# TUI-NICR/nicr-multitask-scene-analysis

Hardware: AMD Instinct MI355X
Metric: Mpix/s panoptic merge+metrics, 640x480xB (higher is better)
Workload: dtype f32; 1 GPU; configs[1]: center-NMS + offset grouping + panoptic merge + mIoU/PQ accumulators (configs[3]); batch_per_gpu=32, global_batch=32, classes=40, height=480, width=640, centers_per_image=24, batches_in_flight=2, parallelism=dp1 (images sharded, accumulators all-reduced once per run, timed)

## Files before the change

include/nmsa.h:

```cpp
#ifndef NMSA_H
#define NMSA_H

#include <stddef.h>
#include <stdint.h>

#ifdef __cplusplus
extern "C" {
#endif

typedef void* nmsa_stream_t;

enum {
    NMSA_OK = 0,
    NMSA_ERR_ARG = -1,
    NMSA_ERR_LAUNCH = -2,
    NMSA_ERR_WORKSPACE = -3,
    NMSA_ERR_UNSUPPORTED = -4
};

enum { NMSA_F32 = 0, NMSA_BF16 = 1, NMSA_F16 = 2 };
enum { NMSA_U8 = 0, NMSA_I16 = 1, NMSA_I32 = 2, NMSA_I64 = 3 };
#define NMSA_ELEM_F32 8

#define NMSA_MAX_INSTANCE_IDS 256

int nmsa_version(void);
const char* nmsa_strerror(int code);
int nmsa_last_hip_error(void);
int nmsa_device_geometry(int* cus_host, int* xcds_host, size_t* lds_per_cu_host);

size_t nmsa_center_nms_workspace_bytes(int B, int H, int W);
int nmsa_center_nms_topk(const float* center, const uint8_t* fg,
                         int B, int H, int W,
                         float threshold, int ksize, int topk, int apply_fg,
                         int max_centers,
                         int32_t* centers_yx, int32_t* n_centers, float* scores,
                         uint8_t* center_mask,
                         void* workspace, size_t workspace_bytes,
                         nmsa_stream_t stream);

int nmsa_group_offsets(const float* offset, const uint8_t* fg,
                       const int32_t* centers_yx, const int32_t* n_centers,
                       int B, int H, int W, int max_centers,
                       float scale_y, float scale_x,
                       int use_dist_thr, float dist_thr,
                       uint8_t* inst, int32_t* area,
                       nmsa_stream_t stream);

int nmsa_semantic_argmax(const void* logits, int logits_dtype,
                         int B, int C, int H, int W,
                         uint8_t* idx_u8, int64_t* idx_i64, float* score,
                         nmsa_stream_t stream);

int nmsa_semantic_softmax(const void* logits, int logits_dtype,
                          int B, int C, int H, int W, float* probs,
                          nmsa_stream_t stream);

int nmsa_panoptic_fused(const void* logits, int logits_dtype, const float* offset,
                        const int32_t* centers_yx, const int32_t* n_centers,
                        const uint8_t* is_thing,
                        int B, int C, int H, int W, int max_centers,
                        float scale_y, float scale_x,
                        int use_dist_thr, float dist_thr,
                        uint8_t* sem_u8, uint8_t* inst, uint8_t* fg_out, float* score,
                        uint32_t* votes, int votes_are_zero, int vote_rows_hint,
                        nmsa_stream_t stream);

int nmsa_panoptic_assign(uint32_t* votes, int B, int n_vote_classes, int clear_votes,
                         int64_t max_instances_per_category, int64_t void_label,
                         int64_t* pan_of_inst, int32_t* area,
                         int64_t* ids_pan, int64_t* ids_ins, int32_t* n_ids,
                         nmsa_stream_t stream);

int nmsa_panoptic_paint(const uint8_t* sem_u8, const uint8_t* inst,
                        const int64_t* pan_of_inst, const uint8_t* is_thing,
                        int B, int C, int H, int W,
                        int64_t max_instances_per_category, int64_t void_label,
                        int64_t* pan, int64_t* pan_sem,
                        nmsa_stream_t stream);

int nmsa_panoptic_merge(const void* sem, int sem_dtype, const void* ins, int ins_dtype,
                        const uint8_t* thing_seg, const uint8_t* is_thing_class,
                        int B, int n_classes, int H, int W,
                        int64_t max_instances_per_category, int64_t void_label,
                        uint32_t* votes, int64_t* pan_of_inst,
                        int64_t* pan, int64_t* ids_pan, int64_t* ids_ins, int32_t* n_ids,
                        nmsa_stream_t stream);

size_t nmsa_panoptic_merge_wide_workspace_bytes(int B, int n_classes, int max_segments);
int nmsa_panoptic_merge_wide(const void* sem, int sem_dtype, const void* ins, int ins_dtype,
                             const uint8_t* thing_seg, const uint8_t* is_thing_class,
                             int B, int n_classes, int H, int W,
// ... 387 lines not shown
```

nicr_mt_scene_analysis_amd/_lib.py:

```python
import ctypes as C
import os
import re
import subprocess
from typing import Optional

import torch

_HERE = os.path.dirname(os.path.abspath(__file__))
CSRC_DIR = os.path.join(_HERE, 'csrc')
LIB_PATH = os.environ.get('NMSA_LIB_PATH') or os.path.join(CSRC_DIR, 'libnmsa_hip.so')
HEADER_PATH = os.path.join(os.path.dirname(_HERE), 'include', 'nmsa.h')

NMSA_F32, NMSA_BF16, NMSA_F16 = 0, 1, 2
NMSA_U8, NMSA_I16, NMSA_I32, NMSA_I64 = 0, 1, 2, 3
NMSA_ST_VALUE_RANGE = 8
NMSA_SCENE_MAX_CLASSES = 4096
(NMSA_TG_ROUTE_SCAN, NMSA_TG_ROUTE_FAST_LOADERS, NMSA_TG_ROUTE_PAINT_TILED, NMSA_TG_ROUTE_PAINT_VECTOR,
 NMSA_TG_ROUTE_LUT_LDS, NMSA_TG_ROUTE_SCAN_16) = 1, 2, 4, 8, 16, 32
NMSA_UP_ROUTE_VECTOR, NMSA_UP_ROUTE_PIXEL = 1, 2
NMSA_LNT_ROUTE_VECTOR, NMSA_LNT_ROUTE_ELEMENT = 1, 2
NMSA_LNT_MAX_CHANNELS = 2048


class NmsaError(RuntimeError):
    pass


def build(force: bool = False) -> str:
    args = ['make', '-C', CSRC_DIR, '-j4']
    if force:
        args.append('-B')
    subprocess.check_call(args, stdout=subprocess.DEVNULL)
    return LIB_PATH


def declared_symbols():
    with open(HEADER_PATH) as f:
        text = f.read()
    text = re.sub(r'/\*.*?\*/', '', text, flags=re.S)
    return sorted(set(re.findall(r'\b(nmsa_[a-z0-9_]+)\s*\(', text)))


_vp, _i, _f, _i64, _sz = C.c_void_p, C.c_int, C.c_float, C.c_int64, C.c_size_t

_SIGNATURES = {
    'nmsa_version': (C.c_int, []),
    'nmsa_strerror': (C.c_char_p, [_i]),
    'nmsa_last_hip_error': (C.c_int, []),
    'nmsa_device_geometry': (_i, [_vp, _vp, _vp]),
    'nmsa_center_nms_workspace_bytes': (_sz, [_i, _i, _i]),
    'nmsa_center_nms_topk': (_i, [_vp, _vp, _i, _i, _i, _f, _i, _i, _i, _i,
                                  _vp, _vp, _vp, _vp, _vp, _sz, _vp]),
    'nmsa_group_offsets': (_i, [_vp, _vp, _vp, _vp, _i, _i, _i, _i, _f, _f, _i, _f,
                                _vp, _vp, _vp]),
    'nmsa_semantic_argmax': (_i, [_vp, _i, _i, _i, _i, _i, _vp, _vp, _vp, _vp]),
    'nmsa_semantic_softmax': (_i, [_vp, _i, _i, _i, _i, _i, _vp, _vp]),
    'nmsa_panoptic_fused': (_i, [_vp, _i, _vp, _vp, _vp, _vp, _i, _i, _i, _i, _i,
                                 _f, _f, _i, _f, _vp, _vp, _vp, _vp, _vp, _i, _i, _vp]),
    'nmsa_panoptic_assign': (_i, [_vp, _i, _i, _i, _i64, _i64, _vp, _vp, _vp, _vp, _vp, _vp]),
    'nmsa_panoptic_paint': (_i, [_vp, _vp, _vp, _vp, _i, _i, _i, _i, _i64, _i64,
                                 _vp, _vp, _vp]),
    'nmsa_panoptic_merge': (_i, [_vp, _i, _vp, _i, _vp, _vp, _i, _i, _i, _i, _i64, _i64,
                                 _vp, _vp, _vp, _vp, _vp, _vp, _vp]),
    'nmsa_panoptic_merge_wide_workspace_bytes': (_sz, [_i, _i, _i]),
    'nmsa_panoptic_merge_wide': (_i, [_vp, _i, _vp, _i, _vp, _vp, _i, _i, _i, _i, _i64, _i64, _i,
                                      _vp, _vp, _vp, _vp, _vp, _vp, _sz, _vp]),
    'nmsa_resize_nearest': (_i, [_vp, _i, _i, _i, _i, _i, _i, _i, _i, _i, _i, _vp, _vp]),
    'nmsa_resize_bilinear': (_i, [_vp, _i, _i, _i, _i, _i, _i, _i, _i, _i, _i, _vp, _vp]),
    'nmsa_semantic_argmax_resized': (_i, [_vp, _i, _i, _i, _i, _i, _i, _i, _i, _i, _i, _i,
                                          _vp, _vp, _vp, _vp]),
    'nmsa_panoptic_scores_workspace_bytes': (_sz, [_i]),
    'nmsa_panoptic_scores': (_i, [_vp, _i, _vp, _vp, _vp, _vp, _vp, _vp, _i, _i, _i, _i, _i64,
                                  _vp, _vp, _vp, _vp, _vp, _sz, _vp]),
    'nmsa_targets_workspace_bytes': (_sz, [_i, _i, _i]),
    'nmsa_targets_route': (_i, [_vp, _i, _vp, _i, _i, _i, _i, _i, _i, _vp, _vp, _vp, _vp, _vp]),
    'nmsa_instance_clear_stuff': (_i, [_vp, _i, _vp, _i, _vp, _i, _i64, _vp]),
    'nmsa_instance_targets': (_i, [_vp, _i, _vp, _i, _vp, _vp, _i, _i, _i, _i, _i, _vp, _i, _i,
                                   _vp, _vp, _vp, _vp, _vp, _vp, _vp, _vp, _vp, _vp, _sz, _i, _vp]),
    'nmsa_panoptic_targets': (_i, [_vp, _i, _vp, _i, _vp, _i, _i, _i, _i, _i64, _i64, _i, _i,
                                   _vp, _vp, _vp, _vp, _vp, _vp, _sz, _i, _vp]),
    'nmsa_orientation_targets': (_i, [_vp, _i, _vp, _i, _vp, _vp, _vp, _vp, _i, _i, _i, _i, _i, _i,
                                      _vp, _vp, _vp, _vp, _vp, _sz, _i, _vp]),
    'nmsa_dve_targets': (_i, [_vp, _vp, _vp, _vp, _vp, _f, _i, _i, _i, _i, _i, _vp, _vp, _vp]),
    'nmsa_dve_project': (_i, [_vp, _i, _i, _i, _i, _vp, _i, _vp, _vp, _i, _vp, _i, _vp]),
    'nmsa_dve_project_route': (_i, [_vp, _i, _i, _i, _i, _vp, _i, _vp, _vp, _i, _vp, _i]),
    'nmsa_normal_valid_mask': (_i, [_vp, _i, _i, _i, _vp, _vp]),
    'nmsa_rmse_update': (_i, [_vp, _i, _vp, _vp, _i, _i, _i, _i, _i, _i, _i, _i, _i, _i, _i,
                              _vp, _vp, _vp]),
    'nmsa_maae_update_keyed': (_i, [_vp, _vp, _vp, _vp, _i, _vp, _vp, _vp, _vp, _vp, _i, _vp,
                                    _i, _vp, _vp, _vp, _vp]),
    'nmsa_maae_update_matched': (_i, [_vp, _vp, _i, _vp, _vp, _vp, _i, _i, _vp, _vp, _vp, _vp, _i, _vp,
                                      _vp, _vp, _vp, _i, _i, _vp, _vp, _vp, _vp, _i, _vp,
                                      _i, _vp, _vp, _vp, _vp]),
    'nmsa_multiscale_nearest': (_i, [_vp, _vp, _i, _i, _vp]),
    'nmsa_batch_augment': (_i, [_vp, _vp, _i, _i, _i, _vp]),
    'nmsa_scene_step': (_i, [_vp, _i, _vp, _i, _i, _i, _vp, _f, _vp, _vp, _vp, _vp, _vp, _vp, _vp]),
    'nmsa_upsample2x_dw3x3_route': (_i, [_vp, _vp, _i, _i, _i, _i, _i]),
    'nmsa_upsample2x_dw3x3_fwd': (_i, [_vp, _i, _vp, _vp, _i, _i, _i, _i, _i, _vp, _vp]),
    'nmsa_upsample2x_dw3x3_bwd_workspace_bytes': (_sz, [_i, _i, _i, _i]),
    'nmsa_upsample2x_dw3x3_bwd': (_i, [_vp, _vp, _i, _vp, _i, _i, _i, _i, _i, _vp, _vp, _vp, _vp, _sz, _vp]),
    'nmsa_ln_nhwc_nchw_route': (_i, [_vp, _vp, _i, _i, _i, _i, _i]),
    'nmsa_ln_nhwc_nchw_fwd': (_i, [_vp, _i, _vp, _vp, _f, _vp, _i, _i, _i, _vp, _i, _vp, _vp, _vp]),
    'nmsa_ln_nhwc_nchw_bwd_workspace_bytes': (_sz, [_i, _i, _i]),
    'nmsa_ln_nhwc_nchw_bwd': (_i, [_vp, _i, _vp, _i, _vp, _vp, _vp, _i, _i, _i, _vp, _vp, _vp, _vp, _sz, _vp]),
    'nmsa_instance_orientation_wide': (_i, [_vp, _vp, _i, _vp, _i, _i, _i, _i, _vp, _vp, _vp, _vp,
# ... 4 lines not shown
    'nmsa_pq_confmat_workspace_bytes': (_sz, [_i, _i, _i, _i]),
    'nmsa_pq_update_with_confmat': (_i, [_vp, _vp, _vp, _i, _i, _i, _i, _i64, _i64, _i64, _i64,
                                         _vp, _vp, _vp, _vp, _vp, _i, _vp, _vp, _vp, _sz, _i,
                                         _i, _i64, _vp, _vp, _vp, _sz, _vp]),
    'nmsa_pq_update_with_confmat_parts': (_i, [_vp, _vp, _vp, _vp, _i, _i64, _vp, _vp, _i, _i, _i,
                                               _i, _i64, _i64, _i64, _i64, _vp, _vp, _vp, _vp,
                                               _vp, _vp, _sz, _i, _i, _i64, _vp, _vp, _vp, _sz, _vp]),
    'nmsa_pack_tables': (_i, [_vp, _vp, _vp, _vp, _vp, _vp, _vp, _i, _i, _i, _vp, _vp]),
    'nmsa_loss_workspace_bytes': (_sz, [_i, _i, _i]),
    'nmsa_loss_ce_fwd': (_i, [_vp, _i, _vp, _vp, _i, _i, _i, _i, _f, _vp, _vp, _vp, _vp, _vp, _vp, _sz,
                              _vp]),
    'nmsa_loss_ce_bwd': (_i, [_vp, _i, _vp, _vp, _i, _i, _i, _i, _f, _vp, _vp, _vp, _vp]),
    'nmsa_loss_ce_fwd_i16': (_i, [_vp, _i, _vp, _vp, _i, _i, _i, _i, _f, _vp, _vp, _vp, _vp, _vp, _vp, _sz,
                                  _vp]),
    'nmsa_loss_ce_bwd_i16': (_i, [_vp, _i, _vp, _vp, _i, _i, _i, _i, _f, _vp, _vp, _vp, _vp]),
    'nmsa_loss_masked_fwd': (_i, [_vp, _i, _vp, _vp, _i, _i, _i, _i, _i, _vp, _vp, _vp, _sz, _vp]),
    'nmsa_loss_masked_bwd': (_i, [_vp, _i, _vp, _vp, _i, _i, _i, _i, _i, _vp, _vp, _vp]),
    'nmsa_loss_vonmises_fwd': (_i, [_vp, _i, _vp, _vp, _i, _i, _i, _f, _vp, _vp, _vp, _sz, _vp]),
    'nmsa_loss_vonmises_bwd': (_i, [_vp, _i, _vp, _vp, _i, _i, _i, _f, _vp, _vp, _vp]),
    'nmsa_loss_ce_fwd_grad_supported': (_i, [_i, _i]),
    'nmsa_loss_ce_fwd_grad': (_i, [_vp, _i, _vp, _vp, _i, _i, _i, _i, _f, _vp, _vp, _vp, _vp, _vp, _vp,
                                   _vp, _sz, _vp]),
    'nmsa_loss_ce_bwd_unless': (_i, [_vp, _i, _vp, _vp, _i, _i, _i, _i, _f, _vp, _vp, _vp, _vp, _vp]),
    'nmsa_count_workspace_bytes': (_sz, []),
    'nmsa_count_u8': (_i, [_vp, _i64, _i, _i, _vp, _vp, _f, _vp, _sz, _vp]),
    'nmsa_loss_cos_emb_fwd_grad_supported': (_i, [_i, _i, _i, _i, _i]),
    'nmsa_loss_cos_emb_fwd_grad_workspace_bytes': (_sz, [_i, _i, _i, _i, _i]),
    'nmsa_loss_cos_emb_fwd_grad': (_i, [_vp, _i, _vp, _vp, _i, _i, _i, _i, _i, _vp, _vp, _vp, _vp, _vp, _vp, _sz, _vp]),
    'nmsa_loss_cos_emb_bwd_unless': (_i, [_vp, _i, _vp, _vp, _i, _i, _i, _i, _i, _vp, _vp, _vp, _vp, _vp, _sz, _vp]),
    'nmsa_multitask_loss_workspace_bytes': (_sz, [_vp, _i]),
    'nmsa_multitask_loss_fwd_grad': (_i, [_vp, _i, _i, _vp, _vp, _vp, _vp, _vp, _vp, _vp, _vp, _sz, _vp]),
    'nmsa_multitask_loss_bwd_unless': (_i, [_vp, _i, _i, _vp, _vp, _vp, _vp, _vp, _vp, _vp, _vp, _vp, _sz, _vp]),
    'nmsa_loss_masked_fwd_grad': (_i, [_vp, _i, _vp, _vp, _i, _i, _i, _i, _i, _vp, _vp, _vp, _vp, _vp,
                                       _sz, _vp]),
    'nmsa_loss_masked_bwd_unless': (_i, [_vp, _i, _vp, _vp, _i, _i, _i, _i, _i, _vp, _vp, _vp, _vp,
                                         _vp]),
    'nmsa_loss_vonmises_fwd_grad': (_i, [_vp, _i, _vp, _vp, _i, _i, _i, _f, _vp, _vp, _vp, _vp, _vp,
                                         _sz, _vp]),
    'nmsa_loss_vonmises_bwd_unless': (_i, [_vp, _i, _vp, _vp, _i, _i, _i, _f, _vp, _vp, _vp, _vp, _vp]),
    'nmsa_loss_cos_emb_fwd': (_i, [_vp, _i, _vp, _vp, _i, _i, _i, _i, _i, _vp, _vp, _vp, _vp, _vp, _sz, _vp]),
    'nmsa_loss_cos_emb_bwd': (_i, [_vp, _i, _vp, _vp, _i, _i, _i, _i, _i, _vp, _vp, _vp, _vp]),
    'nmsa_loss_cos_emb_can_keep_dots': (_i, [_i, _i, _i, _i]),
    'nmsa_loss_elementwise_none_fwd': (_i, [_vp, _i, _vp, _i64, _i, _i, _vp, _vp]),
    'nmsa_loss_elementwise_none_bwd': (_i, [_vp, _i, _vp, _i64, _i, _i, _vp, _vp, _vp]),
    'nmsa_loss_cos_rows_fwd': (_i, [_vp, _i, _vp, _vp, _i64, _i, _f, _vp, _vp]),
    'nmsa_loss_cos_rows_bwd': (_i, [_vp, _i, _vp, _vp, _i64, _i, _f, _vp, _i, _vp, _vp]),
    'nmsa_loss_vonmises_rows_fwd': (_i, [_vp, _i, _vp, _i64, _f, _vp, _vp]),
    'nmsa_loss_vonmises_rows_bwd': (_i, [_vp, _i, _vp, _i64, _f, _vp, _vp, _vp]),
    'nmsa_pq_workspace_bytes': (_sz, [_i, _i, _i, _i]),
    'nmsa_pq_update': (_i, [_vp, _vp, _i, _i, _i, _i, _i64, _i64, _i64, _i64,
                            _vp, _vp, _vp, _vp, _vp, _i, _vp, _vp, _vp, _sz, _i, _vp]),
}

_lib = None


def lib():
    global _lib
    if _lib is None:
        if not os.path.exists(LIB_PATH):
            raise NmsaError(
                f'{LIB_PATH} is missing: the HIP extension was not built. Run '
                '`python -c "import __graft_entry__ as g; g.build()"` '
                '(or `make -C nicr_mt_scene_analysis_amd/csrc`). There is no '
                'CPU/PyTorch fallback for this path.')
        handle = C.CDLL(LIB_PATH)
        for name, (res, args) in _SIGNATURES.items():
            fn = getattr(handle, name)
            fn.restype = res
            fn.argtypes = args
        _lib = handle
    return _lib


def check(rc: int, what: str) -> None:
    if rc != 0:
        l_ = lib()
        msg = l_.nmsa_strerror(rc).decode()
        hip = l_.nmsa_last_hip_error()
        raise NmsaError(f'{what}: {msg} (code {rc}, hipError {hip})')


def device_geometry():
    cus, xcds, lds = C.c_int(0), C.c_int(0), C.c_size_t(0)
    check(lib().nmsa_device_geometry(C.byref(cus), C.byref(xcds), C.byref(lds)), 'nmsa_device_geometry')
    return cus.value, xcds.value, lds.value


def ptr(t: Optional[torch.Tensor]):
    if t is None:
        return None
    if not t.is_cuda and not t.is_pinned():
        raise ValueError(f'the C-ABI takes device (or pinned host) memory; got a pageable '
                         f'{t.device} tensor of shape {tuple(t.shape)}')
    return C.c_void_p(t.data_ptr())


def stream_ptr(device) -> C.c_void_p:
    return C.c_void_p(torch.cuda.current_stream(device).cuda_stream)


def float_dtype_code(t: torch.Tensor) -> int:
    if t.dtype == torch.float32:
        return NMSA_F32
    if t.dtype == torch.bfloat16:
        return NMSA_BF16
    if t.dtype == torch.float16:
        return NMSA_F16
    raise TypeError(f'unsupported floating dtype {t.dtype}')


def int_dtype_code(t: torch.Tensor) -> int:
    if t.dtype in (torch.uint8, torch.bool):
        return NMSA_U8
    if t.dtype == torch.int16:
        return NMSA_I16
    if t.dtype == torch.int32:
        return NMSA_I32
    if t.dtype == torch.int64:
        return NMSA_I64
# ... 10 lines not shown
```

nicr_mt_scene_analysis_amd/csrc/center_nms.hip:

```cpp
#include <stdlib.h>
#include "nmsa_common.hpp"

namespace nmsa {

constexpr int NMS_TW = 64;
constexpr int NMS_TH = 16;
constexpr int NMS_PAD_MAX = 4;

__device__ __forceinline__ float threshold_m1(float x, float thr)
{
    return (x <= thr) ? -1.0f : x;
}

template <bool USE_LDS>
__global__ __launch_bounds__(256) void k_nms_candidates(
    const float* __restrict__ center, uint32_t* __restrict__ cand_bits,
    int H, int W, int words_per_image, float thr, int pad)
{
    __shared__ float tile[USE_LDS ? (NMS_TH + 2 * NMS_PAD_MAX) * (NMS_TW + 2 * NMS_PAD_MAX) : 1];
    const int b = blockIdx.z;
    const int x0 = blockIdx.x * NMS_TW, y0 = blockIdx.y * NMS_TH;
    const float* img = center + (size_t)b * H * W;
    const int tw = NMS_TW + 2 * pad, th = NMS_TH + 2 * pad;

// ... 80 lines not shown
    uint32_t* bits = cand_bits + (size_t)b * words_per_image;
    constexpr int K = 2 * PAD + 1;
    for (int xb = 0; xb < W; xb += blockDim.x) {
        const int x = xb + threadIdx.x;
        const bool in_x = x < W;
        const int xc = in_x ? x : 0;
        float win[K][K];
#pragma unroll
        for (int i = 0; i < K - 1; ++i)
#pragma unroll
            for (int j = 0; j < K; ++j)
                win[i + 1][j] = strip[i * tw + xc + j];
        for (int r = 0; r < rows; ++r) {
            const int y = y0 + r;
#pragma unroll
            for (int i = 0; i < K - 1; ++i)
#pragma unroll
                for (int j = 0; j < K; ++j) win[i][j] = win[i + 1][j];
#pragma unroll
            for (int j = 0; j < K; ++j) win[K - 1][j] = strip[(r + K - 1) * tw + xc + j];
            bool cand = false;
            if (in_x) {
                const float h = win[PAD][PAD];
                bool survive;
                if (y < PAD || y >= H - PAD || x < PAD || x >= W - PAD) {
                    survive = (y * W + x == 0) && (h == 0.0f);
                } else {
                    survive = true;
#pragma unroll
                    for (int i = 0; i < K; ++i)
#pragma unroll
                        for (int j = 0; j < K; ++j) {
                            if (i == PAD && j == PAD) continue;
                            const bool before = (i < PAD) || (i == PAD && j < PAD);
                            survive = survive && (before ? (win[i][j] < h) : (win[i][j] <= h));
                        }
                    survive = survive && (h == h);
                }
                cand = survive && h >= 0.0f;
            }
            const unsigned long long m = __ballot(cand);
            if (lane_id() == 0) {
                const int x_wave = xb + (int)(threadIdx.x & ~63u);
                if (x_wave < W) {
                    const int word = (y * W + x_wave) >> 5;
                    bits[word] = (uint32_t)m;
                    if (x_wave + 32 < W) bits[word + 1] = (uint32_t)(m >> 32);
                }
            }
        }
    }
}


template <int NR_ROWS, bool HALF>
__global__ __launch_bounds__(256) void k_nms_rows3(
    const float* __restrict__ center, uint32_t* __restrict__ cand_bits,
    int H, int W, int words_per_image, float thr, int blocks_per_image, int n_blocks, int n_xcd)
{
    constexpr int LPB = HALF ? 32 : 64;
    constexpr int BW = LPB * 4;
    const int per_xcd = n_blocks > 0 ? (n_blocks + n_xcd - 1) / n_xcd : 0;
    const int logical = n_blocks > 0 ? (int)(blockIdx.x % n_xcd) * per_xcd + (int)(blockIdx.x / n_xcd) : (int)blockIdx.x;
    if (n_blocks > 0 && logical >= n_blocks) return;
    const int b = n_blocks > 0 ? logical / blocks_per_image : (int)blockIdx.y;
    const int bx = n_blocks > 0 ? logical - b * blocks_per_image : (int)blockIdx.x;
    const int lane = lane_id();
    const int l = lane & (LPB - 1);
    const int sub = HALF ? (lane >> 5) : 0;
    const int bands = (W + BW - 1) / BW;
    const int wave = bx * 4 + (int)(threadIdx.x >> 6);
    const int seg = wave / bands, band = wave - seg * bands;
    const int y0 = (seg * (HALF ? 2 : 1) + sub) * NR_ROWS;
    if ((seg * (HALF ? 2 : 1)) * NR_ROWS >= H) return;
    const int xb = band * BW;
    const int x0 = xb + 4 * l;
    const bool in_x = x0 < W && y0 < H;
    const float* img = center + (size_t)b * H * W;
    const int xe = (l == 0) ? xb - 1 : xb + BW;
    const bool edge_lane = (l == 0 || l == LPB - 1) && xe >= 0 && xe < W;

    float4 row[NR_ROWS + 2];
    float edge[NR_ROWS + 2];
#pragma unroll
    for (int r = 0; r < NR_ROWS + 2; ++r) {
        const int gy = min(max(y0 - 1 + r, 0), H - 1);
        row[r] = in_x ? *(const float4*)(img + (size_t)gy * W + x0) : make_float4(-1.f, -1.f, -1.f, -1.f);
        edge[r] = edge_lane ? img[(size_t)gy * W + xe] : -1.f;
    }
    auto extend = [&](int r, float e[6]) {
        const float4 v = row[r];
        e[1] = threshold_m1(v.x, thr); e[2] = threshold_m1(v.y, thr);
        e[3] = threshold_m1(v.z, thr); e[4] = threshold_m1(v.w, thr);
        const float ev = threshold_m1(edge[r], thr);
        const float lf = __shfl_up(e[4], 1), rr = __shfl_down(e[1], 1);
        e[0] = (l == 0) ? ev : lf;
        e[5] = (l == LPB - 1) ? ev : rr;
    };
    uint32_t* bits = cand_bits + (size_t)b * words_per_image;
    auto hmax3 = [](const float e[6], float hm[4]) {
#pragma unroll
        for (int j = 0; j < 4; ++j) hm[j] = fmaxf(fmaxf(e[j], e[j + 1]), e[j + 2]);
    };
    float top[6], mid[6], bot[6], htop[4], hmid[4], hbot[4];
    extend(0, mid);
    hmax3(mid, hmid);
    extend(1, bot);
    hmax3(bot, hbot);
#pragma unroll
    for (int r = 1; r <= NR_ROWS; ++r) {
        const int y = y0 + r - 1;
#pragma unroll
        for (int k = 0; k < 6; ++k) { top[k] = mid[k]; mid[k] = bot[k]; }
#pragma unroll
        for (int k = 0; k < 4; ++k) { htop[k] = hmid[k]; hmid[k] = hbot[k]; }
        extend(r + 1, bot);
        hmax3(bot, hbot);
        if (__all(y >= H)) break;
        const bool row_ok = y < H;
        const bool border_y = y < 1 || y >= H - 1;
        bool maybe[4];
        bool any_maybe = false;
#pragma unroll
        for (int j = 0; j < 4; ++j) {
            const float h = mid[j + 1];
            const float pooled = fmaxf(fmaxf(htop[j], hmid[j]), hbot[j]);
            maybe[j] = in_x && row_ok && h >= 0.0f &&
                       (border_y || h == pooled || x0 + j < 1 || x0 + j >= W - 1);
            any_maybe = any_maybe || maybe[j];
        }
        uint32_t nib = 0;
        if (__any(any_maybe)) {
#pragma unroll
            for (int j = 0; j < 4; ++j) {
                const int x = x0 + j;
                const float h = mid[j + 1];
                bool survive;
                if (border_y || x < 1 || x >= W - 1) {
                    survive = (y * W + x == 0) && (h == 0.0f);
                } else {
                    survive = (top[j] < h) && (top[j + 1] < h) && (top[j + 2] < h) && (mid[j] < h) &&
                              (mid[j + 2] <= h) && (bot[j] <= h) && (bot[j + 1] <= h) &&
                              (bot[j + 2] <= h) && (h == h);
                }
                if (maybe[j] && survive) nib |= 1u << j;
            }
        }
        uint32_t word = nib << (4 * (lane & 7));
        word |= __shfl_xor(word, 1);
        word |= __shfl_xor(word, 2);
        word |= __shfl_xor(word, 4);
        if ((lane & 7) == 0 && in_x && row_ok) bits[(y * W + x0) >> 5] = word;
    }
}

__device__ __forceinline__ int wave_inclusive_scan(int v)
{
#pragma unroll
    for (int o = 1; o < 64; o <<= 1) {
        const int t = __shfl_up(v, o);
        if (lane_id() >= o) v += t;
    }
    return v;
}

__device__ __forceinline__ int block_inclusive_scan(int v, int* scratch, int* total)
{
    const int w = threadIdx.x >> 6, nw = blockDim.x >> 6;
    const int incl = wave_inclusive_scan(v);
    __syncthreads();
    if (lane_id() == 63) scratch[w] = incl;
    __syncthreads();
    if (w == 0) {
        int s = (lane_id() < nw) ? scratch[lane_id()] : 0;
        s = wave_inclusive_scan(s);
        if (lane_id() < nw) scratch[lane_id()] = s;
    }
    __syncthreads();
    const int base = (w == 0) ? 0 : scratch[w - 1];
    *total = scratch[nw - 1];
    return incl + base;
}

__device__ __forceinline__ uint32_t cand_key(float v)
{
    return (v == 0.0f) ? 0u : __float_as_uint(v);
}

constexpr int SEL_THREADS = 1024;
constexpr int SEL_BINS = 2048;

constexpr int SEL_LDS_WORDS = 36 * 1024;
constexpr int SEL_LIST_CAP = 2048;

template <bool LDS_BITS>
__global__ __launch_bounds__(SEL_THREADS) void k_select_compact(
    const float* __restrict__ center, const uint8_t* __restrict__ fg,
    const uint32_t* __restrict__ cand_bits,
    int H, int W, int words_per_image, int topk, int apply_fg, int max_centers,
    int32_t* __restrict__ centers_yx, int32_t* __restrict__ n_centers,
    float* __restrict__ scores, uint8_t* __restrict__ center_mask, int list_cap)
{
    __shared__ int hist[SEL_BINS];
    __shared__ int scratch[32];
    __shared__ uint32_t s_prefix;
    __shared__ int s_krem;
// ... 119 lines not shown
            keep |= k ? (1u << (e - e0)) : 0u;
        }
        const int mine_l = __popc(keep);
        int n_total_l;
        const int incl_l = block_inclusive_scan(mine_l, scratch, &n_total_l);
        int pos_l = incl_l - mine_l;
        for (int e = e0; e < e1; ++e) {
            if (!((keep >> (e - e0)) & 1u)) continue;
            const int p = (int)s_lpos[e];
            if (pos_l < max_centers) {
                const int y = p / W;
                centers_yx[((size_t)b * max_centers + pos_l) * 2 + 0] = y;
                centers_yx[((size_t)b * max_centers + pos_l) * 2 + 1] = p - y * W;
                scores[(size_t)b * max_centers + pos_l] = img[p];
            }
            if (center_mask) center_mask[(size_t)b * P + p] = 1;
            ++pos_l;
        }
        if (threadIdx.x == 0) n_centers[b] = n_total_l;
        return;
    }
    int mine = 0;
    for (int w = w_begin; w < w_end; ++w) {
        uint32_t m = bits[w];
        while (m) {
            const int bit = __ffs((int)m) - 1;
            m &= m - 1;
            mine += kept((w << 5) + bit) ? 1 : 0;
        }
    }
    int n_total;
    const int incl = block_inclusive_scan(mine, scratch, &n_total);
    int pos = incl - mine;
    for (int w = w_begin; w < w_end; ++w) {
        uint32_t m = bits[w];
        while (m) {
            const int bit = __ffs((int)m) - 1;
            m &= m - 1;
            const int p = (w << 5) + bit;
            if (!kept(p)) continue;
            if (pos < max_centers) {
                const int y = p / W;
                centers_yx[((size_t)b * max_centers + pos) * 2 + 0] = y;
                centers_yx[((size_t)b * max_centers + pos) * 2 + 1] = p - y * W;
                scores[(size_t)b * max_centers + pos] = img[p];
            }
            if (center_mask) center_mask[(size_t)b * P + p] = 1;
            ++pos;
        }
    }
    if (threadIdx.x == 0) n_centers[b] = n_total;
}

}

using namespace nmsa;

extern "C" size_t nmsa_center_nms_workspace_bytes(int B, int H, int W)
{
    if (B <= 0 || H <= 0 || W <= 0) return 0;
    const size_t words = ((size_t)H * W + 31) / 32;
    return (size_t)B * words * sizeof(uint32_t);
}

extern "C" int nmsa_center_nms_topk(const float* center, const uint8_t* fg,
                                    int B, int H, int W,
                                    float threshold, int ksize, int topk, int apply_fg,
                                    int max_centers,
                                    int32_t* centers_yx, int32_t* n_centers, float* scores,
                                    uint8_t* center_mask,
                                    void* workspace, size_t workspace_bytes,
                                    nmsa_stream_t stream_)
{
    hipStream_t stream = (hipStream_t)stream_;
    if (!center || !centers_yx || !n_centers || !scores || !workspace) return NMSA_ERR_ARG;
    if (B <= 0 || H <= 0 || W <= 0 || max_centers <= 0) return NMSA_ERR_ARG;
    if (ksize < 1 || (ksize & 1) == 0 || topk < 1) return NMSA_ERR_ARG;
    if ((int64_t)H * W > (int64_t)1 << 30) return NMSA_ERR_ARG;
    if ((int64_t)H * W < topk) return NMSA_ERR_ARG;
    if (apply_fg && !fg) return NMSA_ERR_ARG;
    if (workspace_bytes < nmsa_center_nms_workspace_bytes(B, H, W)) return NMSA_ERR_WORKSPACE;

    const int words = (int)(((size_t)H * W + 31) / 32);
    uint32_t* bits = (uint32_t*)workspace;
    int rc;
    if (center_mask) {
        rc = check_hip(hipMemsetAsync(center_mask, 0, (size_t)B * H * W, stream));
        if (rc) return rc;
    }
    const int pad = (ksize - 1) / 2;
    static const int rows_env = getenv("NMSA_NMS_ROWS") ? atoi(getenv("NMSA_NMS_ROWS")) : 0;
    int R = rows_env > 0 ? rows_env : 4;
    while (R > 1 && (size_t)(R + 2 * pad) * (W + 2 * pad) * sizeof(float) > 48 * 1024) R >>= 1;
    const size_t strip_lds = (size_t)(R + 2 * pad) * (W + 2 * pad) * sizeof(float);
    static const int rows3_env = getenv("NMSA_NMS_ROWS3") ? atoi(getenv("NMSA_NMS_ROWS3")) : 1;
    if (pad == 1 && (W % 32) == 0 && rows3_env) {
        static const int nr = getenv("NMSA_NMS_NR") ? atoi(getenv("NMSA_NMS_NR")) : 4;
        static const int half_env = getenv("NMSA_NMS_HALF") ? atoi(getenv("NMSA_NMS_HALF")) : -1;
        const bool half = half_env >= 0 ? (half_env != 0 && W % 128 == 0) : (W % 256 != 0 && W % 128 == 0);
        static const int xcd = getenv("NMSA_NMS_XCD") ? atoi(getenv("NMSA_NMS_XCD")) : 1;
        const int nx = device_geometry().xcds;
#define NMSA_ROWS3(NR) do {                                                                                 \
        const int waves = half ? (W / 128) * ((H + 2 * NR - 1) / (2 * NR)) : ((W + 255) / 256) * ((H + NR - 1) / NR); \
        const int bpi = (waves + 3) / 4;                                                                    \
        const long long nb = (long long)bpi * B;                                                            \
        const bool remap = xcd && nx > 1 && nb < (1ll << 30);                                               \
        const dim3 grid_ = remap ? dim3((unsigned)(((nb + nx - 1) / nx) * nx)) : dim3(bpi, B);              \
        if (half) hipLaunchKernelGGL((k_nms_rows3<NR, true>), grid_, dim3(256), 0, stream, center, bits, H, W, \
                                     words, threshold, bpi, remap ? (int)nb : 0, nx);                        \
        else hipLaunchKernelGGL((k_nms_rows3<NR, false>), grid_, dim3(256), 0, stream, center, bits, H, W,   \
                                words, threshold, bpi, remap ? (int)nb : 0, nx); } while (0)
        if (nr == 8) NMSA_ROWS3(8); else NMSA_ROWS3(4);
#undef NMSA_ROWS3
    } else if ((W % 32) == 0 && pad <= NMS_PAD_MAX && strip_lds <= 64 * 1024) {
        dim3 grid((H + R - 1) / R, B);
        static const int thr_env = getenv("NMSA_NMS_THREADS") ? atoi(getenv("NMSA_NMS_THREADS")) : 0;
        const int strip_threads = thr_env > 0 ? thr_env : 256;
#define NMSA_STRIP(PADV) hipLaunchKernelGGL(k_nms_strip<PADV>, grid, dim3(strip_threads), strip_lds, stream, \
                                            center, bits, H, W, R, words, threshold)
        switch (pad) {
            case 0: NMSA_STRIP(0); break;
            case 1: NMSA_STRIP(1); break;
            case 2: NMSA_STRIP(2); break;
            case 3: NMSA_STRIP(3); break;
            default: NMSA_STRIP(4); break;
        }
#undef NMSA_STRIP
    } else {
        rc = check_hip(hipMemsetAsync(bits, 0, (size_t)B * words * sizeof(uint32_t), stream));
        if (rc) return rc;
        dim3 grid((W + NMS_TW - 1) / NMS_TW, (H + NMS_TH - 1) / NMS_TH, B);
        if (pad <= NMS_PAD_MAX)
            hipLaunchKernelGGL(k_nms_candidates<true>, grid, dim3(256), 0, stream,
                               center, bits, H, W, words, threshold, pad);
        else
            hipLaunchKernelGGL(k_nms_candidates<false>, grid, dim3(256), 0, stream,
                               center, bits, H, W, words, threshold, pad);
    }
    rc = check_launch();
    if (rc) return rc;
    const int list_cap = (words + 2 * SEL_LIST_CAP <= SEL_LDS_WORDS) ? SEL_LIST_CAP : 0;
    const size_t sel_lds = ((size_t)words + 2 * (size_t)list_cap) * sizeof(uint32_t);
    if (words <= SEL_LDS_WORDS &&
        (sel_lds <= 48 * 1024 ||
         allow_dynamic_lds(k_select_compact<true>, SEL_LDS_WORDS * sizeof(uint32_t)) == NMSA_OK)) {
        hipLaunchKernelGGL(k_select_compact<true>, dim3(B), dim3(SEL_THREADS), sel_lds,
                           stream, center, apply_fg ? fg : nullptr, bits, H, W, words, topk, apply_fg,
                           max_centers, centers_yx, n_centers, scores, center_mask, list_cap);
    } else {
        hipLaunchKernelGGL(k_select_compact<false>, dim3(B), dim3(SEL_THREADS), 0, stream,
                           center, apply_fg ? fg : nullptr, bits, H, W, words, topk, apply_fg,
                           max_centers, centers_yx, n_centers, scores, center_mask, 0);
    }
    return check_launch();
}
```

nicr_mt_scene_analysis_amd/ops.py:

```python
import math
from typing import Dict, Optional, Sequence, Tuple

import numpy as np
import torch

from . import _lib as L

DEFAULT_MAX_CENTERS = 256

_VOTE_TABLES: 'collections.OrderedDict[tuple, torch.Tensor]' = __import__('collections').OrderedDict()
_VOTE_TABLES_MAX = 8


def _vote_table(dev: torch.device, B: int, n_cols: int) -> torch.Tensor:
    key = (dev, B, n_cols, torch.cuda.current_stream(dev).cuda_stream)
    t = _VOTE_TABLES.get(key)
    if t is None:
        t = torch.zeros((B, 256, n_cols), dtype=torch.int32, device=dev)
        _VOTE_TABLES[key] = t
        while len(_VOTE_TABLES) > _VOTE_TABLES_MAX:
            _VOTE_TABLES.popitem(last=False)
    else:
        _VOTE_TABLES.move_to_end(key)
    return t


def _u8(t: Optional[torch.Tensor]) -> Optional[torch.Tensor]:
    if t is None:
        return None
    if t.dtype == torch.bool:
        return t.contiguous().view(torch.uint8)
    if t.dtype == torch.uint8:
        return t.contiguous()
    return (t != 0).contiguous().view(torch.uint8)


def center_nms_topk(
    center_heatmap: torch.Tensor,
    foreground_mask: Optional[torch.Tensor] = None,
    threshold: float = 0.1,
    kernel_size: int = 3,
    top_k: int = 64,
    apply_foreground_mask: bool = False,
    max_centers: int = DEFAULT_MAX_CENTERS,
    want_mask: bool = False,
) -> Dict[str, torch.Tensor]:
    c = L.require_device_tensor(center_heatmap, 'center_heatmap')
    if c.dtype != torch.float32:
        c = c.float()
    if c.ndim == 4:
        assert c.shape[1] == 1
        c = c[:, 0]
    c = c.contiguous()
    B, H, W = c.shape
    dev = c.device
    fg = _u8(foreground_mask) if apply_foreground_mask else None
    cyx = torch.empty((B, max_centers, 2), dtype=torch.int32, device=dev)
    n = torch.empty((B,), dtype=torch.int32, device=dev)
    scores = torch.empty((B, max_centers), dtype=torch.float32, device=dev)
    mask = torch.empty((B, H, W), dtype=torch.uint8, device=dev) if want_mask else None
    ws_bytes = L.lib().nmsa_center_nms_workspace_bytes(B, H, W)
    ws = torch.empty((ws_bytes,), dtype=torch.uint8, device=dev)
    L.check(L.lib().nmsa_center_nms_topk(
        L.ptr(c), L.ptr(fg), B, H, W, float(threshold), int(kernel_size), int(top_k),
        int(bool(apply_foreground_mask)), int(max_centers),
        L.ptr(cyx), L.ptr(n), L.ptr(scores), L.ptr(mask), L.ptr(ws), ws_bytes,
        L.stream_ptr(dev)), 'nmsa_center_nms_topk')
    out = {'centers_yx': cyx, 'n_centers': n, 'scores': scores}
    if want_mask:
        out['center_mask'] = mask.view(torch.bool)
    return out


def group_offsets(
    center_offset: torch.Tensor,
    foreground_mask: torch.Tensor,
    centers_yx: torch.Tensor,
    n_centers: torch.Tensor,
    scale_y: float = 1.0,
    scale_x: float = 1.0,
    distance_threshold: Optional[float] = None,
    want_area: bool = True,
) -> Dict[str, torch.Tensor]:
    off = L.require_device_tensor(center_offset, 'center_offset')
    if off.dtype != torch.float32:
        off = off.float()
    B, two, H, W = off.shape
    assert two == 2
    dev = off.device
    fg = _u8(foreground_mask)
    inst = torch.empty((B, H, W), dtype=torch.uint8, device=dev)
    area = torch.empty((B, 256), dtype=torch.int32, device=dev) if want_area else None
    L.check(L.lib().nmsa_group_offsets(
        L.ptr(off), L.ptr(fg), L.ptr(centers_yx), L.ptr(n_centers), B, H, W,
        int(centers_yx.shape[1]), float(scale_y), float(scale_x),
        0 if distance_threshold is None else 1,
        0.0 if distance_threshold is None else float(distance_threshold),
        L.ptr(inst), L.ptr(area), L.stream_ptr(dev)), 'nmsa_group_offsets')
    return {'instance': inst, 'area': area}


NMSA_ELEM_F32 = 8


def _crop_geometry(t: torch.Tensor, crop) -> Tuple[int, int, int, int, int, int]:
    Hs, Ws = int(t.shape[-2]), int(t.shape[-1])
    if crop is None:
        return Hs, Ws, 0, 0, Hs, Ws
    sl_h, sl_w = crop
    y0, y1, st_y = sl_h.indices(Hs)
    x0, x1, st_x = sl_w.indices(Ws)
    if st_y != 1 or st_x != 1 or y1 <= y0 or x1 <= x0:
        raise ValueError(f'unsupported valid-region slices {crop}')
    return Hs, Ws, y0, x0, y1 - y0, x1 - x0


def resize_nearest(maps: torch.Tensor, size: Tuple[int, int], crop=None) -> torch.Tensor:
    x = L.require_device_tensor(maps, 'maps')
    code = NMSA_ELEM_F32 if x.dtype == torch.float32 else L.int_dtype_code(x)
    Hs, Ws, y0, x0, h, w = _crop_geometry(x, crop)
# ... 1217 lines not shown
```

Measured before the change: 32080 Mpix/s.

## Fuse center-NMS candidate pass with top-k selection via last-block ticket tail

Merges the row-wise NMS kernel and the separate top-k select/compact kernel into one launch. Each block publishes its candidate bits with atomic stores and takes a per-image ticket. The last block to finish an image runs the radix-select and compaction tail for that image. This removes one kernel launch and the gap between launches, but the whole selection for an image now runs in a single 256-thread block and needs a persistent, zero-initialised ticket buffer per stream.

After: 31520 Mpix/s. -1.7%, worse.

```diff
diff --git a/include/nmsa.h b/include/nmsa.h
--- a/include/nmsa.h
+++ b/include/nmsa.h
@@ -38,6 +38,16 @@
                          uint8_t* center_mask,
                          void* workspace, size_t workspace_bytes,
                          nmsa_stream_t stream);
+size_t nmsa_center_nms_tickets_bytes(int B);
+int nmsa_center_nms_topk_tail(const float* center, const uint8_t* fg,
+                              int B, int H, int W,
+                              float threshold, int ksize, int topk, int apply_fg,
+                              int max_centers,
+                              int32_t* centers_yx, int32_t* n_centers, float* scores,
+                              uint8_t* center_mask,
+                              void* workspace, size_t workspace_bytes,
+                              void* tickets, size_t tickets_bytes,
+                              nmsa_stream_t stream);
 
 int nmsa_group_offsets(const float* offset, const uint8_t* fg,
                        const int32_t* centers_yx, const int32_t* n_centers,
diff --git a/nicr_mt_scene_analysis_amd/_lib.py b/nicr_mt_scene_analysis_amd/_lib.py
--- a/nicr_mt_scene_analysis_amd/_lib.py
+++ b/nicr_mt_scene_analysis_amd/_lib.py
@@ -51,6 +51,9 @@
     'nmsa_center_nms_workspace_bytes': (_sz, [_i, _i, _i]),
     'nmsa_center_nms_topk': (_i, [_vp, _vp, _i, _i, _i, _f, _i, _i, _i, _i,
                                   _vp, _vp, _vp, _vp, _vp, _sz, _vp]),
+    'nmsa_center_nms_tickets_bytes': (_sz, [_i]),
+    'nmsa_center_nms_topk_tail': (_i, [_vp, _vp, _i, _i, _i, _f, _i, _i, _i, _i,
+                                       _vp, _vp, _vp, _vp, _vp, _sz, _vp, _sz, _vp]),
     'nmsa_group_offsets': (_i, [_vp, _vp, _vp, _vp, _i, _i, _i, _i, _f, _f, _i, _f,
                                 _vp, _vp, _vp]),
     'nmsa_semantic_argmax': (_i, [_vp, _i, _i, _i, _i, _i, _vp, _vp, _vp, _vp]),
@@ -161,6 +164,8 @@
                             _vp, _vp, _vp, _vp, _vp, _i, _vp, _vp, _vp, _sz, _i, _vp]),
 }
 
+_NEWER_ENTRY_POINTS = ('nmsa_center_nms_tickets_bytes', 'nmsa_center_nms_topk_tail')
+
 _lib = None
 
 
@@ -175,6 +180,8 @@
                 'CPU/PyTorch fallback for this path.')
         handle = C.CDLL(LIB_PATH)
         for name, (res, args) in _SIGNATURES.items():
+            if name in _NEWER_ENTRY_POINTS and os.environ.get('NMSA_LIB_PATH') and not hasattr(handle, name):
+                continue
             fn = getattr(handle, name)
             fn.restype = res
             fn.argtypes = args
diff --git a/nicr_mt_scene_analysis_amd/csrc/center_nms.hip b/nicr_mt_scene_analysis_amd/csrc/center_nms.hip
--- a/nicr_mt_scene_analysis_amd/csrc/center_nms.hip
+++ b/nicr_mt_scene_analysis_amd/csrc/center_nms.hip
@@ -156,19 +156,24 @@
     }
 }
 
-
-template <int NR_ROWS, bool HALF>
-__global__ __launch_bounds__(256) void k_nms_rows3(
-    const float* __restrict__ center, uint32_t* __restrict__ cand_bits,
-    int H, int W, int words_per_image, float thr, int blocks_per_image, int n_blocks, int n_xcd)
+__device__ __forceinline__ bool rows3_locate(int blocks_per_image, int n_blocks, int n_xcd, int* b, int* bx)
+{
+    const int per_xcd = n_blocks > 0 ? (n_blocks + n_xcd - 1) / n_xcd : 0;
+    const int logical = n_blocks > 0 ? (int)(blockIdx.x % n_xcd) * per_xcd + (int)(blockIdx.x / n_xcd) : (int)blockIdx.x;
+    if (n_blocks > 0 && logical >= n_blocks) return false;
+    *b = n_blocks > 0 ? logical / blocks_per_image : (int)blockIdx.y;
+    *bx = n_blocks > 0 ? logical - *b * blocks_per_image : (int)blockIdx.x;
+    return true;
+}
+
+
+template <int NR_ROWS, bool HALF, bool PUBLISH>
+__device__ __forceinline__ void nms_rows3_body(
+    const float* __restrict__ center, uint32_t* cand_bits,
+    int H, int W, int words_per_image, float thr, int b, int bx)
 {
     constexpr int LPB = HALF ? 32 : 64;
     constexpr int BW = LPB * 4;
-    const int per_xcd = n_blocks > 0 ? (n_blocks + n_xcd - 1) / n_xcd : 0;
-    const int logical = n_blocks > 0 ? (int)(blockIdx.x % n_xcd) * per_xcd + (int)(blockIdx.x / n_xcd) : (int)blockIdx.x;
-    if (n_blocks > 0 && logical >= n_blocks) return;
-    const int b = n_blocks > 0 ? logical / blocks_per_image : (int)blockIdx.y;
-    const int bx = n_blocks > 0 ? logical - b * blocks_per_image : (int)blockIdx.x;
     const int lane = lane_id();
     const int l = lane & (LPB - 1);
     const int sub = HALF ? (lane >> 5) : 0;
@@ -254,8 +259,21 @@
         word |= __shfl_xor(word, 1);
         word |= __shfl_xor(word, 2);
         word |= __shfl_xor(word, 4);
-        if ((lane & 7) == 0 && in_x && row_ok) bits[(y * W + x0) >> 5] = word;
-    }
+        if ((lane & 7) == 0 && in_x && row_ok) {
+            if (PUBLISH) __hip_atomic_store(&bits[(y * W + x0) >> 5], word, __ATOMIC_RELAXED, __HIP_MEMORY_SCOPE_AGENT);
+            else bits[(y * W + x0) >> 5] = word;
+        }
+    }
+}
+
+template <int NR_ROWS, bool HALF>
+__global__ __launch_bounds__(256) void k_nms_rows3(
+    const float* __restrict__ center, uint32_t* __restrict__ cand_bits,
+    int H, int W, int words_per_image, float thr, int blocks_per_image, int n_blocks, int n_xcd)
+{
+    int b, bx;
+    if (!rows3_locate(blocks_per_image, n_blocks, n_xcd, &b, &bx)) return;
+    nms_rows3_body<NR_ROWS, HALF, false>(center, cand_bits, H, W, words_per_image, thr, b, bx);
 }
 
 __device__ __forceinline__ int wave_inclusive_scan(int v)
@@ -481,6 +499,190 @@
     if (threadIdx.x == 0) n_centers[b] = n_total;
 }
 
+constexpr int NMS_TICKET_STRIDE = 64;
+constexpr int TAIL_THREADS = 256;
+constexpr int TAIL_BINS_PER_THREAD = SEL_BINS / TAIL_THREADS;
+
+struct SelTailLds {
+    int hist[SEL_BINS];
+    uint32_t lpos[SEL_LIST_CAP];
+    uint32_t lkey[SEL_LIST_CAP];
+    int scratch[32];
+    uint32_t prefix;
+    int krem;
+    int last;
+};
+
+__device__ __forceinline__ void select_tail(
+    SelTailLds& S, const float* __restrict__ img, const uint8_t* __restrict__ fgb, const uint32_t* bits,
+    int b, int H, int W, int words_per_image, int topk, int apply_fg, int max_centers,
+    int32_t* __restrict__ centers_yx, int32_t* __restrict__ n_centers, float* __restrict__ scores,
+    uint8_t* __restrict__ center_mask)
+{
+    const int t = threadIdx.x;
+    const int P = H * W;
+    const int wpt = (words_per_image + TAIL_THREADS - 1) / TAIL_THREADS;
+    const int w_begin = min(t * wpt, words_per_image);
+    const int w_end = min(w_begin + wpt, words_per_image);
+    auto walk = [&](auto&& fn) {
+        for (int w0 = w_begin; w0 < w_end; w0 += 8) {
+            uint32_t m[8];
+#pragma unroll
+            for (int u = 0; u < 8; ++u) m[u] = (w0 + u < w_end) ? bits[w0 + u] : 0u;
+#pragma unroll
+            for (int u = 0; u < 8; ++u) {
+                uint32_t x = m[u];
+                while (x) {
+                    const int bit = __ffs((int)x) - 1;
+                    x &= x - 1;
+                    fn(((w0 + u) << 5) + bit);
+                }
+            }
+        }
+    };
+
+    int cnt = 0;
+    for (int w0 = w_begin; w0 < w_end; w0 += 8) {
+        uint32_t m[8];
+#pragma unroll
+        for (int u = 0; u < 8; ++u) m[u] = (w0 + u < w_end) ? bits[w0 + u] : 0u;
+#pragma unroll
+        for (int u = 0; u < 8; ++u) cnt += __popc(m[u]);
+    }
+    int total;
+    const int cnt_incl = block_inclusive_scan(cnt, S.scratch, &total);
+
+    const bool use_list = total <= SEL_LIST_CAP;
+    if (use_list) {
+        int at = cnt_incl - cnt;
+        walk([&](int p) {
+            S.lpos[at] = (uint32_t)p;
+            S.lkey[at] = cand_key(img[p]);
+            ++at;
+        });
+        __syncthreads();
+    }
+
+    uint32_t key_kth = 0;
+    if (total >= topk) {
+        if (t == 0) { S.prefix = 0; S.krem = topk; }
+        const int shifts[3] = {21, 10, 0};
+        const int nbits[3] = {11, 11, 10};
+        for (int pass = 0; pass < 3; ++pass) {
+            const int shift = shifts[pass];
+            const int nb = 1 << nbits[pass];
+            for (int i = t; i < SEL_BINS; i += TAIL_THREADS) S.hist[i] = 0;
+            __syncthreads();
+            const uint32_t prefix = S.prefix;
+            const int hi_shift = shift + nbits[pass];
+            auto vote = [&](uint32_t k) {
+                const bool match = (hi_shift >= 32) || ((k >> hi_shift) == (prefix >> hi_shift));
+                if (match) atomicAdd(&S.hist[(k >> shift) & (nb - 1)], 1);
+            };
+            if (use_list) {
+                for (int e = t; e < total; e += TAIL_THREADS) vote(S.lkey[e]);
+            } else {
+                walk([&](int p) { vote(cand_key(img[p])); });
+            }
+            __syncthreads();
+            int c[TAIL_BINS_PER_THREAD], sum = 0;
+#pragma unroll
+            for (int j = 0; j < TAIL_BINS_PER_THREAD; ++j) {
+                c[j] = S.hist[SEL_BINS - 1 - (TAIL_BINS_PER_THREAD * t + j)];
+                sum += c[j];
+            }
+            int dummy;
+            const int incl = block_inclusive_scan(sum, S.scratch, &dummy);
+            int above = incl - sum;
+            const int krem = S.krem;
+            __syncthreads();
+            if (above < krem && krem <= incl) {
+                int sel = 0, new_k = 0;
+                bool found = false;
+#pragma unroll
+                for (int j = 0; j < TAIL_BINS_PER_THREAD; ++j) {
+                    if (!found && above + c[j] >= krem) {
+                        sel = SEL_BINS - 1 - (TAIL_BINS_PER_THREAD * t + j);
+                        new_k = krem - above;
+                        found = true;
+                    }
+                    above += c[j];
+                }
+                S.prefix = prefix | ((uint32_t)sel << shift);
+                S.krem = new_k;
+            }
+            __syncthreads();
+        }
+        key_kth = S.prefix;
+    }
+
+    auto emit = [&](int p, int pos) {
+        if (pos < max_centers) {
+            const int y = p / W;
+            centers_yx[((size_t)b * max_centers + pos) * 2 + 0] = y;
+            centers_yx[((size_t)b * max_centers + pos) * 2 + 1] = p - y * W;
+            scores[(size_t)b * max_centers + pos] = img[p];
+        }
+        if (center_mask) center_mask[(size_t)b * P + p] = 1;
+    };
+    int n_total;
+    if (use_list) {
+        const int per = (total + TAIL_THREADS - 1) / TAIL_THREADS;
+        const int e0 = min(t * per, total), e1 = min(e0 + per, total);
+        uint32_t keep = 0u;
+        for (int e = e0; e < e1; ++e) {
+            const bool k = S.lkey[e] >= key_kth && (!apply_fg || fgb[S.lpos[e]]);
+            keep |= k ? (1u << (e - e0)) : 0u;
+        }
+        const int mine = __popc(keep);
+        int pos = block_inclusive_scan(mine, S.scratch, &n_total) - mine;
+        for (int e = e0; e < e1; ++e)
+            if ((keep >> (e - e0)) & 1u) emit((int)S.lpos[e], pos++);
+    } else {
+        auto kept = [&](int p) -> bool {
+            if (apply_fg && !fgb[p]) return false;
+            return cand_key(img[p]) >= key_kth;
+        };
+        int mine = 0;
+        walk([&](int p) { mine += kept(p) ? 1 : 0; });
+        int pos = block_inclusive_scan(mine, S.scratch, &n_total) - mine;
+        walk([&](int p) { if (kept(p)) emit(p, pos++); });
+    }
+    if (t == 0) n_centers[b] = n_total;
+}
+
+template <int NR_ROWS, bool HALF>
+__global__ __launch_bounds__(TAIL_THREADS) void k_nms_rows3_select(
+    const float* __restrict__ center, const uint8_t* __restrict__ fg, uint32_t* cand_bits,
+    int H, int W, int words_per_image, float thr, int blocks_per_image, int n_blocks, int n_xcd,
+    int topk, int apply_fg, int max_centers,
+    int32_t* __restrict__ centers_yx, int32_t* __restrict__ n_centers, float* __restrict__ scores,
+    uint8_t* __restrict__ center_mask, unsigned int* tickets)
+{
+    __shared__ SelTailLds S;
+    int b, bx;
+    if (!rows3_locate(blocks_per_image, n_blocks, n_xcd, &b, &bx)) return;
+    nms_rows3_body<NR_ROWS, HALF, true>(center, cand_bits, H, W, words_per_image, thr, b, bx);
+    asm volatile("s_waitcnt vmcnt(0)" ::: "memory");
+    __syncthreads();
+    unsigned int* ticket = tickets + (size_t)b * NMS_TICKET_STRIDE;
+    if (threadIdx.x == 0) {
+        const bool last = atomicAdd(ticket, 1u) == (unsigned)blocks_per_image - 1u;
+        S.last = last ? 1 : 0;
+        if (last) {
+            __builtin_amdgcn_fence(__ATOMIC_ACQUIRE, "agent");
+            asm volatile("s_waitcnt vmcnt(0)" ::: "memory");
+        }
+    }
+    __syncthreads();
+    if (!S.last) return;
+    const size_t P = (size_t)H * W;
+    select_tail(S, center + (size_t)b * P, fg ? fg + (size_t)b * P : nullptr,
+                cand_bits + (size_t)b * words_per_image, b, H, W, words_per_image, topk, apply_fg,
+                max_centers, centers_yx, n_centers, scores, center_mask);
+    if (threadIdx.x == 0) __hip_atomic_store(ticket, 0u, __ATOMIC_RELAXED, __HIP_MEMORY_SCOPE_AGENT);
+}
+
 }
 
 using namespace nmsa;
@@ -492,14 +694,19 @@
     return (size_t)B * words * sizeof(uint32_t);
 }
 
-extern "C" int nmsa_center_nms_topk(const float* center, const uint8_t* fg,
-                                    int B, int H, int W,
-                                    float threshold, int ksize, int topk, int apply_fg,
-                                    int max_centers,
-                                    int32_t* centers_yx, int32_t* n_centers, float* scores,
-                                    uint8_t* center_mask,
-                                    void* workspace, size_t workspace_bytes,
-                                    nmsa_stream_t stream_)
+extern "C" size_t nmsa_center_nms_tickets_bytes(int B)
+{
+    return B > 0 ? (size_t)B * NMS_TICKET_STRIDE * sizeof(uint32_t) : 0;
+}
+
+static int center_nms_topk_impl(const float* center, const uint8_t* fg,
+                                int B, int H, int W,
+                                float threshold, int ksize, int topk, int apply_fg,
+                                int max_centers,
+                                int32_t* centers_yx, int32_t* n_centers, float* scores,
+                                uint8_t* center_mask,
+                                void* workspace, size_t workspace_bytes,
+                                unsigned int* tickets, nmsa_stream_t stream_)
 {
     hipStream_t stream = (hipStream_t)stream_;
     if (!center || !centers_yx || !n_centers || !scores || !workspace) return NMSA_ERR_ARG;
@@ -529,18 +736,28 @@
         const bool half = half_env >= 0 ? (half_env != 0 && W % 128 == 0) : (W % 256 != 0 && W % 128 == 0);
         static const int xcd = getenv("NMSA_NMS_XCD") ? atoi(getenv("NMSA_NMS_XCD")) : 1;
         const int nx = device_geometry().xcds;
+        const char* tail_env = tickets ? getenv("NMSA_NMS_TAIL") : nullptr;
+        const bool tail = tickets && !(tail_env && atoi(tail_env) == 0);
 #define NMSA_ROWS3(NR) do {                                                                                 \
         const int waves = half ? (W / 128) * ((H + 2 * NR - 1) / (2 * NR)) : ((W + 255) / 256) * ((H + NR - 1) / NR); \
         const int bpi = (waves + 3) / 4;                                                                    \
         const long long nb = (long long)bpi * B;                                                            \
         const bool remap = xcd && nx > 1 && nb < (1ll << 30);                                               \
         const dim3 grid_ = remap ? dim3((unsigned)(((nb + nx - 1) / nx) * nx)) : dim3(bpi, B);              \
-        if (half) hipLaunchKernelGGL((k_nms_rows3<NR, true>), grid_, dim3(256), 0, stream, center, bits, H, W, \
+        if (tail) {                                                                                         \
+            if (half) hipLaunchKernelGGL((k_nms_rows3_select<NR, true>), grid_, dim3(TAIL_THREADS), 0, stream, \
+                center, apply_fg ? fg : nullptr, bits, H, W, words, threshold, bpi, remap ? (int)nb : 0, nx, \
+                topk, apply_fg, max_centers, centers_yx, n_centers, scores, center_mask, tickets);          \
+            else hipLaunchKernelGGL((k_nms_rows3_select<NR, false>), grid_, dim3(TAIL_THREADS), 0, stream,  \
+                center, apply_fg ? fg : nullptr, bits, H, W, words, threshold, bpi, remap ? (int)nb : 0, nx, \
+                topk, apply_fg, max_centers, centers_yx, n_centers, scores, center_mask, tickets);          \
+        } else if (half) hipLaunchKernelGGL((k_nms_rows3<NR, true>), grid_, dim3(256), 0, stream, center, bits, H, W, \
                                      words, threshold, bpi, remap ? (int)nb : 0, nx);                        \
         else hipLaunchKernelGGL((k_nms_rows3<NR, false>), grid_, dim3(256), 0, stream, center, bits, H, W,   \
                                 words, threshold, bpi, remap ? (int)nb : 0, nx); } while (0)
         if (nr == 8) NMSA_ROWS3(8); else NMSA_ROWS3(4);
 #undef NMSA_ROWS3
+        if (tail) return check_launch();
     } else if ((W % 32) == 0 && pad <= NMS_PAD_MAX && strip_lds <= 64 * 1024) {
         dim3 grid((H + R - 1) / R, B);
         static const int thr_env = getenv("NMSA_NMS_THREADS") ? atoi(getenv("NMSA_NMS_THREADS")) : 0;
@@ -583,3 +800,34 @@
     }
     return check_launch();
 }
+
+extern "C" int nmsa_center_nms_topk(const float* center, const uint8_t* fg,
+                                    int B, int H, int W,
+                                    float threshold, int ksize, int topk, int apply_fg,
+                                    int max_centers,
+                                    int32_t* centers_yx, int32_t* n_centers, float* scores,
+                                    uint8_t* center_mask,
+                                    void* workspace, size_t workspace_bytes,
+                                    nmsa_stream_t stream)
+{
+    return center_nms_topk_impl(center, fg, B, H, W, threshold, ksize, topk, apply_fg, max_centers,
+                                centers_yx, n_centers, scores, center_mask, workspace, workspace_bytes,
+                                nullptr, stream);
+}
+
+extern "C" int nmsa_center_nms_topk_tail(const float* center, const uint8_t* fg,
+                                         int B, int H, int W,
+                                         float threshold, int ksize, int topk, int apply_fg,
+                                         int max_centers,
+                                         int32_t* centers_yx, int32_t* n_centers, float* scores,
+                                         uint8_t* center_mask,
+                                         void* workspace, size_t workspace_bytes,
+                                         void* tickets, size_t tickets_bytes,
+                                         nmsa_stream_t stream)
+{
+    if (!tickets) return NMSA_ERR_ARG;
+    if (B > 0 && tickets_bytes < nmsa_center_nms_tickets_bytes(B)) return NMSA_ERR_WORKSPACE;
+    return center_nms_topk_impl(center, fg, B, H, W, threshold, ksize, topk, apply_fg, max_centers,
+                                centers_yx, n_centers, scores, center_mask, workspace, workspace_bytes,
+                                (unsigned int*)tickets, stream);
+}
diff --git a/nicr_mt_scene_analysis_amd/ops.py b/nicr_mt_scene_analysis_amd/ops.py
--- a/nicr_mt_scene_analysis_amd/ops.py
+++ b/nicr_mt_scene_analysis_amd/ops.py
@@ -22,6 +22,22 @@
             _VOTE_TABLES.popitem(last=False)
     else:
         _VOTE_TABLES.move_to_end(key)
+    return t
+
+
+_NMS_TICKETS: 'collections.OrderedDict[tuple, torch.Tensor]' = __import__('collections').OrderedDict()
+
+
+def _nms_tickets(dev: torch.device, B: int) -> torch.Tensor:
+    key = (dev, B, torch.cuda.current_stream(dev).cuda_stream)
+    t = _NMS_TICKETS.get(key)
+    if t is None:
+        t = torch.zeros((L.lib().nmsa_center_nms_tickets_bytes(B),), dtype=torch.uint8, device=dev)
+        _NMS_TICKETS[key] = t
+        while len(_NMS_TICKETS) > _VOTE_TABLES_MAX:
+            _NMS_TICKETS.popitem(last=False)
+    else:
+        _NMS_TICKETS.move_to_end(key)
     return t
 
 
@@ -61,11 +77,15 @@
     mask = torch.empty((B, H, W), dtype=torch.uint8, device=dev) if want_mask else None
     ws_bytes = L.lib().nmsa_center_nms_workspace_bytes(B, H, W)
     ws = torch.empty((ws_bytes,), dtype=torch.uint8, device=dev)
-    L.check(L.lib().nmsa_center_nms_topk(
-        L.ptr(c), L.ptr(fg), B, H, W, float(threshold), int(kernel_size), int(top_k),
-        int(bool(apply_foreground_mask)), int(max_centers),
-        L.ptr(cyx), L.ptr(n), L.ptr(scores), L.ptr(mask), L.ptr(ws), ws_bytes,
-        L.stream_ptr(dev)), 'nmsa_center_nms_topk')
+    args = (L.ptr(c), L.ptr(fg), B, H, W, float(threshold), int(kernel_size), int(top_k),
+            int(bool(apply_foreground_mask)), int(max_centers),
+            L.ptr(cyx), L.ptr(n), L.ptr(scores), L.ptr(mask), L.ptr(ws), ws_bytes)
+    if hasattr(L.lib(), 'nmsa_center_nms_topk_tail'):
+        tickets = _nms_tickets(dev, B)
+        L.check(L.lib().nmsa_center_nms_topk_tail(*args, L.ptr(tickets), tickets.numel(),
+                                                  L.stream_ptr(dev)), 'nmsa_center_nms_topk_tail')
+    else:
+        L.check(L.lib().nmsa_center_nms_topk(*args, L.stream_ptr(dev)), 'nmsa_center_nms_topk')
     out = {'centers_yx': cyx, 'n_centers': n, 'scores': scores}
     if want_mask:
         out['center_mask'] = mask.view(torch.bool)
```
